# criteo-research/reco-gym

Hardware: AMD Instinct MI355X
Metric: env steps/sec (organic+bandit events emitted/sec), reco-gym-v1 P=10000 K=20 (higher is better)
Workload: dtype f64 (state, click, transition, policy, propensities); organic logits on MFMA as a 2-way fp16 split of fp32 operands (fp32 accumulate), every index certified against f64; 1 GPU; c3: reco-gym-v1 P=10000 K=20 sigma_omega=0.0 policy=ouc; users_per_gpu=10000000, users_total=10000000, log=16 B/row device log + float64 ps side array

## Files before the change

### __graft_entry__.py

```python
import glob
import os
import subprocess
import sys

ROOT = os.path.dirname(os.path.abspath(__file__))
if ROOT not in sys.path:
    sys.path.insert(0, ROOT)

HIPCC = os.environ.get('HIPCC', '/opt/rocm/bin/hipcc')


def _stale(out, deps):
    return (not os.path.exists(out)) or any(os.path.getmtime(d) > os.path.getmtime(out) for d in deps)


UNITS = ['rg_host', 'rg_exact', 'rg_draw_fp32', 'rg_draw_pipelined', 'rg_draw_wide', 'rg_advance', 'rg_walk', 'rg_draw_exacthi', 'rg_draw_lds', 'rg_ope', 'rg_count', 'rg_ope_logreg', 'rg_ope_eg', 'rg_evolve', 'rg_logreg_poly', 'rg_ope_poly', 'rg_ope_recall', 'rg_weight_history', 'rg_bayes_vb', 'rg_nn_ips']
N_PARTS = len(UNITS)
UNIT_FLAGS = {'rg_draw_lds': ['-mllvm', '-amdgpu-mfma-vgpr-form=1']}


def build_deps():
    return sorted(glob.glob(os.path.join(ROOT, 'recogym_amd', 'csrc', '*.hpp')) + glob.glob(os.path.join(ROOT, 'include', '*.h')))


def build(force=False, parts=None, extra_flags=(), out=None):
    csrc = os.path.join(ROOT, 'recogym_amd', 'csrc')
    srcs = [os.path.join(csrc, u + '.hip') for u in UNITS]
    default_out = os.path.join(csrc, 'librecogym_hip.so')
    out = out or default_out
    objdir = os.path.join(csrc, 'build' if out == default_out else 'build_' + os.path.basename(out).replace('.so', ''))
    deps = srcs + build_deps()
    if force or parts or _stale(out, deps):
        os.makedirs(objdir, exist_ok=True)
        todo = list(parts) if parts else list(range(1, N_PARTS + 1))
        for p in range(1, N_PARTS + 1):
            if p not in todo and _stale(os.path.join(objdir, f'part{p}.o'), deps):
                todo.append(p)
        procs = []
        for p in todo:
            cmd = [HIPCC, '--offload-arch=gfx950', '-O3', '-std=c++17', '-fPIC', *UNIT_FLAGS.get(UNITS[p - 1], []), *extra_flags, '-c',
                   '-o', os.path.join(objdir, f'part{p}.o'), srcs[p - 1]]
            procs.append((p, subprocess.Popen(cmd, stderr=open(os.path.join(objdir, f'part{p}.log'), 'w'))))
        for p, pr in procs:
            if pr.wait() != 0:
                sys.stderr.write(open(os.path.join(objdir, f'part{p}.log')).read()[-8000:])
                raise RuntimeError(f'hipcc failed on {UNITS[p - 1]}.hip')
        subprocess.check_call([HIPCC, '--offload-arch=gfx950', '-shared', '-fPIC', '-o', out] +
                              [os.path.join(objdir, f'part{p}.o') for p in range(1, N_PARTS + 1)])
    from oracle import oracle as orc
    orc.build(force=force)
    import recogym_amd
    from recogym_amd import _abi
    _abi.load()
    return out


def smoke():
    import numpy as np
    import torch
    build()
    from oracle import oracle as orc
    from recogym_amd import _abi
    from recogym_amd.envs.configuration import Configuration
    from recogym_amd.envs.reco_env_v1 import env_1_args
    from recogym_amd.sim import Simulator
    assert torch.cuda.is_available(), 'smoke() needs a GPU'
    cfg = Configuration({**env_1_args, 'random_seed': 123, 'num_products': 500, 'K': 20})
    n = 2000
    sim = Simulator(cfg, n, device='cuda:0')
    sim.reset_users(0, n)
    sim.run()
    rows = sim.rows()
    want = orc.OracleEnv(cfg, rng_mode=orc.RNG_PHILOX).generate_logs(n)
    assert len(rows) == len(want), (len(rows), len(want))
    for k in ('u', 't', 'z', 'v', 'a', 'c'):
        assert (rows[k].astype(np.int64) == want[k].astype(np.int64)).all(), k
    c = sim.counters()
    print(f'smoke ok: {len(rows)} rows bit-exact vs oracle; counters {c}')


if __name__ == '__main__':
    _parts = [int(x) for x in sys.argv[sys.argv.index('--parts') + 1].split(',')] if '--parts' in sys.argv else None
    build(force='--force' in sys.argv, parts=_parts)
    if '--smoke' in sys.argv:
        smoke()
```

### recogym_amd/csrc/rg_common.hpp

```cpp

#include <hip/hip_runtime.h>

#include <cmath>
#include <cstdarg>
#include <cstdio>
#include <cstdlib>
#include <cstring>
#include <new>
#include <utility>
#include <vector>

#include "../../include/recogym_hip.h"
#include "../../include/recogym_rng.h"

#pragma once

#ifndef RG_WALK_PRECISE_CHUNK
#define RG_WALK_PRECISE_CHUNK 1
#endif

namespace rgk {

constexpr uint32_t kMaxSteps = 1u << 16;
constexpr int kBlock = 256;
constexpr int kMaxGrid = 4096;
constexpr uint32_t kDefaultHistoryCap = 256;
constexpr uint32_t kPolyListCap = 4096;
constexpr uint32_t kPolySteps = 1024;
constexpr uint32_t kPolyHist = 256;
inline bool lr_family(uint32_t policy) { return policy == RG_POLICY_LOGREG_FROZEN || policy == RG_POLICY_LOGREG_POLY || policy == RG_POLICY_BAYES_VB || policy == RG_POLICY_NN_IPS; }
inline bool lists_unresolved(uint32_t policy) { return policy == RG_POLICY_LOGREG_POLY || policy == RG_POLICY_BAYES_VB || policy == RG_POLICY_NN_IPS; }
constexpr uint64_t kBayesModelBytes = 1ull << 31;
constexpr uint32_t kNnHidden = 1024;
constexpr uint32_t kNnProducts = 4000;
constexpr size_t kNnStageBytes = 48 * 1024;
constexpr size_t kNnStaticLds = 16 * 1024;
constexpr uint64_t kRepackMinUsers = 1ull << 18;

inline thread_local char g_err[512] = "";

inline int fail(int code, const char* fmt, ...) {
    va_list ap;
    va_start(ap, fmt);
    vsnprintf(g_err, sizeof(g_err), fmt, ap);
    va_end(ap);
    return code;
}

#define HIP_TRY(expr)                                                                     \
    do {                                                                                  \
        hipError_t e_ = (expr);                                                           \
        if (e_ != hipSuccess)                                                             \
            return fail(RG_ENODEV, "%s failed: %s", #expr, hipGetErrorString(e_));        \
    } while (0)

inline size_t align_up(size_t x, size_t a) { return (x + a - 1) / a * a; }

struct TpRec { double u; float S, pb, q, dlt; uint32_t ti, pad; };
constexpr uint32_t kTpShards = 16, kTpBins = 128, kTpLists = kTpBins * kTpShards;
__host__ __device__ constexpr uint32_t tp_shards_of(uint32_t n_tiles) {
    uint32_t s = kTpShards;
    while (s < 128u && 2u * s * (n_tiles ? n_tiles : 1u) <= kTpLists) s *= 2u;
    return s;
}
__host__ __device__ constexpr uint32_t tp_rec_stride(uint32_t KH) { return (32u + 8u * KH + 63u) & ~63u; }
inline uint32_t tp_shard_cap(uint64_t n, uint32_t shards) { return static_cast<uint32_t>((((n + 255) / 256 + shards - 1) / shards) * 256); }

struct DevSim {
    uint32_t P, K;
    uint64_t seed, policy_seed;
    double cdf_o0, cdf_o1, cdf_b0, cdf_b1;
    double sigma0, sigma_omega;
    uint32_t change_omega_for_bandits, policy;
    uint32_t ouc_select_randomly, ouc_exploit_explore, ouc_reverse_pop, hist_cap;
    double ouc_epsilon;
    uint64_t first_user;
    uint32_t n_users;
    uint32_t n_cap, n_pad;
    uint64_t organic_only_below;
    const double* gamma; const double* mu_o; const double* beta; const double* mu_b;
    float* gamma32; float* mu32;
    uint32_t has_g32t;
    float* gamma32t;
    double* gammaT;
    uint32_t PT;
    double* gamma_rm;
    uint32_t XKB;
    float* exact_ref;
    double* exact_sums;
    uint32_t exact_rows;
    uint32_t walk_handover;
    uint32_t walk_refill;
    uint32_t walk_bias;
    uint32_t walk_click_batch;
    uint32_t walk_search_batch;
    uint32_t walk_helpers;
    uint32_t walk_click_join;
    uint32_t walk_line64;
    uint32_t exact_base;
    uint32_t exact_last;
    float2* sc_scratch;
    float* chunk_scratch;
    char* tp_rec;
    uint32_t* tp_hist;
    uint32_t* tp_order;
    uint32_t tp_cap, tp_shards;
    uint32_t tp_cpt;
    float* stats;
    uint32_t KH;
    uint32_t KS;
    uint32_t TP;
    uint32_t P_pad;
    uint32_t n_chunks;
    uint32_t sc_chunks;
    uint32_t n_sc;
    uint32_t use_mfma;
    uint32_t N1, N2, N3;
    uint32_t f16;
    uint32_t wide;
    uint32_t RS;
    uint32_t TPB;
    unsigned short* gsplit;
    float* mu32s;
    uint32_t XNH, XNL, XRS;
    unsigned short* xsplit;
    float* xmulo;
    float* xstats;
    uint32_t ablate;
    uint32_t use_cache;
    float2* cache_rec;
    float* cache_chunk;
    float* beta32;
    uint32_t KB4;
    uint8_t* cache_resc;
    float* cache_row; uint32_t cache_row_f;
    float* walk_hot; float* walk_scp;
    uint32_t fin_in_sweep;
    uint32_t sweep_only;
    uint32_t* park_list;
    uint32_t* park_t;
    uint8_t* f64_valid;
    uint32_t grp_lo, grp_n;
    uint32_t list_in;
    unsigned long long* q_ticket;
    unsigned long long* q_park;
    const unsigned long long* q_count;
    unsigned long long* walk_ctl;
    unsigned long long* step1_buf;
    uint32_t* exact_cnt_b;
    double* omega;
    uint32_t OMS;
    uint32_t* list;
    uint32_t* step_cnt;
    uint64_t* log_base;
    uint32_t* exact_list;
    uint32_t* exact_cnt;
    uint32_t run_ahead;
    uint32_t* ev;
    unsigned long long* run_ctl;
    uint32_t* n_events;
    rg_event* phantom;
    uint8_t* has_phantom;
    unsigned long long* hist;
    uint32_t* lpv;
    uint32_t* uid;
    double* omega_alt; unsigned long long* hist_alt; uint32_t* lpv_alt; uint32_t* uid_alt;
// ... 869 lines not shown
    *ps_out = 1.0;
    if (d.policy != RG_POLICY_LOGREG_FROZEN) g = policy_act(d, slot, user, t, ps_out);
    return eg_overlay(d, user, t, g, ps_out);
}

__device__ void history_add(const DevSim& d, uint32_t slot, uint32_t v) {
    if (d.lr_dirty) d.lr_dirty[d.uid[slot]] = 1;
    hent_t* hr = hist_row(d, slot);
    hent_t e[kHistRegs];
    hist_load_line(hr, e);
    const uint32_t nd = h_cnt(e[0]);
    const hent_t key = static_cast<hent_t>(v) << 32;
    if (nd < kHistRegs) {
        uint32_t pos = 1;
        bool hit = false;
#pragma unroll
        for (int i = 1; i < kHistRegs; ++i)
            if (static_cast<uint32_t>(i) <= nd) {
                pos += e[i] < key ? 1u : 0u;
                hit = hit || h_prod(e[i]) == v;
            }
        if (hit) {
#pragma unroll
            for (int i = 1; i < kHistRegs; ++i)
                if (static_cast<uint32_t>(i) == pos) hr[i] = e[i] + 1ull;
            hr[0] = e[0] + (1ull << 32);
            return;
        }
        if (nd + 1 >= d.hist_cap) { atomicAdd(&d.counters[RG_CNT_HIST_OVERFLOW], 1ull); return; }
        hent_t f[kHistRegs + 2];
        f[0] = e[0] + (1ull << 32) + 1ull;
#pragma unroll
        for (int i = 1; i < kHistRegs + 1; ++i)
            f[i] = static_cast<uint32_t>(i) < pos ? e[i < kHistRegs ? i : 0] : (static_cast<uint32_t>(i) == pos ? (key | 1ull) : e[i - 1]);
        f[kHistRegs + 1] = 0ull;
        hr[0] = f[0];
#pragma unroll
        for (int i = 0; i < (kHistRegs + 2) / 2; ++i)
            if (static_cast<uint32_t>(2 * i + 1) >= pos && static_cast<uint32_t>(2 * i) <= nd + 1)
                reinterpret_cast<ulonglong2*>(hr)[i] = make_ulonglong2(i == 0 ? f[0] : f[2 * i], f[2 * i + 1]);
        return;
    }
    if RG_WALK_ABL(22) return;
    uint32_t pos = 1;
    hent_t at = 0ull;
    bool past = false;
    for (uint32_t base = 0; base <= nd && !past; base += kHistRegs) {
        hent_t f[kHistRegs];
        if (base) hist_load_line(hr + base, f);
        else {
#pragma unroll
            for (int i = 0; i < kHistRegs; ++i) f[i] = e[i];
        }
#pragma unroll
        for (int i = 0; i < kHistRegs; ++i) {
            const uint32_t idx = base + i;
            if (idx >= 1 && idx <= nd && !past) {
                if (f[i] < key) pos = idx + 1;
                else { past = true; at = f[i]; }
            }
        }
    }
    if (past && h_prod(at) == v) {
        hr[pos] = at + 1ull;
        hr[0] = e[0] + (1ull << 32);
        return;
    }
    if (nd + 1 >= d.hist_cap) { atomicAdd(&d.counters[RG_CNT_HIST_OVERFLOW], 1ull); return; }
    uint32_t j = nd + 1;
    while (j > pos) {
        if (j >= pos + 4) {
            const hent_t a0 = hr[j - 4], a1 = hr[j - 3], a2 = hr[j - 2], a3 = hr[j - 1];
            hr[j - 3] = a0; hr[j - 2] = a1; hr[j - 1] = a2; hr[j] = a3;
            j -= 4;
        } else { hr[j] = hr[j - 1]; --j; }
    }
    hr[pos] = key | 1ull;
    hr[0] = e[0] + (1ull << 32) + 1ull;
}

__device__ __forceinline__ uint32_t history_tail_add(hent_t* hr, uint32_t nd, uint32_t v, uint32_t first = 16u) {
    const hent_t key = static_cast<hent_t>(v) << 32;
    uint32_t pos = first;
    hent_t at = 0ull;
    bool past = false;
    for (uint32_t base = first; base <= nd && !past; base += kHistRegs) {
        hent_t f[kHistRegs];
        hist_load_line(hr + base, f);
#pragma unroll
        for (int i = 0; i < kHistRegs; ++i) {
            const uint32_t idx = base + i;
            if (idx <= nd && !past) {
                if (f[i] < key) pos = idx + 1;
                else { past = true; at = f[i]; }
            }
        }
    }
    if (past && h_prod(at) == v) { hr[pos] = at + 1ull; return 0u; }
    uint32_t j = nd + 1;
    while (j > pos) {
        if (j >= pos + 4) {
            const hent_t a0 = hr[j - 4], a1 = hr[j - 3], a2 = hr[j - 2], a3 = hr[j - 1];
            hr[j - 3] = a0; hr[j - 2] = a1; hr[j - 1] = a2; hr[j] = a3;
            j -= 4;
        } else { hr[j] = hr[j - 1]; --j; }
    }
    hr[pos] = key | 1ull;
    return 1u;
}

__device__ __forceinline__ double wave_max(double x) {
    for (int o = 32; o > 0; o >>= 1) x = fmax(x, __shfl_xor(x, o));
    return x;
}
__device__ __forceinline__ double wave_sum(double x) {
    for (int o = 32; o > 0; o >>= 1) x += __shfl_xor(x, o);
    return x;
}

__device__ __forceinline__ void write_organic_row(const DevSim& d, uint32_t t, uint32_t pos, uint32_t slot,
                                                  uint32_t user, uint32_t v) {
    const uint64_t row = d.log_base[t] + pos;
    if (d.log && row < d.log_cap) {
        rg_event e;
        e.u = user; e.t = d.run_ahead ? d.ev[d.uid[slot]] : t; e.code = v; e.ps = __builtin_nanf("");
        d.log[row] = e;
        if (d.aux_time) d.aux_time[row] = d.utime[d.uid[slot]];
    }
    if (d.lpv) d.lpv[slot] = v;
}

__device__ __forceinline__ double exp64(double x) {
    x = fmax(x, -750.0);
    const double kf = rint(x * 1.4426950408889634074);
    double r = fma(-kf, 6.93147180369123816490e-01, x);
    r = fma(-kf, 1.90821492927058770002e-10, r);
    double p = 1.6059043836821613e-10;
    p = fma(p, r, 2.08767569878681e-09);
    p = fma(p, r, 2.505210838544172e-08);
    p = fma(p, r, 2.755731922398589e-07);
    p = fma(p, r, 2.7557319223985893e-06);
    p = fma(p, r, 2.48015873015873e-05);
    p = fma(p, r, 1.984126984126984e-04);
    p = fma(p, r, 1.388888888888889e-03);
    p = fma(p, r, 8.333333333333333e-03);
    p = fma(p, r, 4.1666666666666664e-02);
    p = fma(p, r, 1.6666666666666666e-01);
    p = fma(p, r, 0.5);
    p = fma(p, r, 1.0);
    p = fma(p, r, 1.0);
    return ldexp(p, static_cast<int>(kf));
}

static __device__ const double kExp2Tab32[32] = {
    0x1.0000000000000p+0, 0x1.059b0d3158574p+0, 0x1.0b5586cf9890fp+0, 0x1.11301d0125b51p+0,
    0x1.172b83c7d517bp+0, 0x1.1d4873168b9aap+0, 0x1.2387a6e756238p+0, 0x1.29e9df51fdee1p+0,
    0x1.306fe0a31b715p+0, 0x1.371a7373aa9cbp+0, 0x1.3dea64c123422p+0, 0x1.44e086061892dp+0,
    0x1.4bfdad5362a27p+0, 0x1.5342b569d4f82p+0, 0x1.5ab07dd485429p+0, 0x1.6247eb03a5585p+0,
    0x1.6a09e667f3bcdp+0, 0x1.71f75e8ec5f74p+0, 0x1.7a11473eb0187p+0, 0x1.82589994cce13p+0,
    0x1.8ace5422aa0dbp+0, 0x1.93737b0cdc5e5p+0, 0x1.9c49182a3f090p+0, 0x1.a5503b23e255dp+0,
    0x1.ae89f995ad3adp+0, 0x1.b7f76f2fb5e47p+0, 0x1.c199bdd85529cp+0, 0x1.cb720dcef9069p+0,
    0x1.d5818dcfba487p+0, 0x1.dfc97337b9b5fp+0, 0x1.ea4afa2a490dap+0, 0x1.f50765b6e4540p+0};

__device__ __forceinline__ double exp64t(double x, const double* tab) {
    x = fmax(x, -750.0);
    const double nf = rint(x * 0x1.71547652b82fep+5);
    double r = fma(nf, -0x1.62e42fe000000p-6, x);
    r = fma(nf, -0x1.f473de6af278fp-35, r);
    const int n = static_cast<int>(nf);
    double p = 1.3888888888888889e-03;
    p = fma(p, r, 8.3333333333333332e-03);
    p = fma(p, r, 4.1666666666666664e-02);
    p = fma(p, r, 1.6666666666666666e-01);
    p = fma(p, r, 0.5);
    p = fma(p, r, 1.0);
    p = fma(p, r, 1.0);
    return ldexp(tab[n & 31] * p, n >> 5);
}

__device__ __forceinline__ double wave_scan(double x, int lane) {
    for (int o = 1; o < 64; o <<= 1) {
        const double y = __shfl_up(x, o);
        if (lane >= o) x += y;
    }
    return x;
}

__device__ __forceinline__ double logit64(const DevSim& d, const double* om, uint32_t p) {
    const double* g = d.gammaT + p;
    double l = 0.0;
#pragma unroll 4
    for (uint32_t k = 0; k < d.K; ++k) l += g[static_cast<size_t>(k) * d.PT] * om[k];
    return l + d.mu_o[p];
}

__device__ __forceinline__ void logit64x4(const DevSim& d, const double* om, uint32_t p, double out[4]) {
    uint32_t idx[4];
#pragma unroll
    for (int u = 0; u < 4; ++u) { idx[u] = min(p + 64u * u, d.PT - 1); out[u] = 0.0; }
#pragma unroll 2
    for (uint32_t k = 0; k < d.K; ++k) {
        const double w = om[k];
        const double* g = d.gammaT + static_cast<size_t>(k) * d.PT;
#pragma unroll
        for (int u = 0; u < 4; ++u) out[u] += g[idx[u]] * w;
    }
#pragma unroll
    for (int u = 0; u < 4; ++u) out[u] = (p + 64u * u < d.P) ? out[u] + d.mu_o[p + 64u * u] : -INFINITY;
}

constexpr int kUPW = 4;
constexpr int kExactUsers = 4 * kUPW;



using f64x4 = __attribute__((ext_vector_type(4))) double;
__host__ __device__ constexpr int exact_m_groups(uint32_t kb) { return kb <= 8 ? 4 : 2; }
__host__ __device__ constexpr uint32_t exact_m_lds(uint32_t kb) { return (2u * 64u * (4u * kb + 4u) + 32u) * 8u; }


typedef const __attribute__((address_space(4))) double kdouble;


inline void launch_exact_m(exact_m_kernel_t km, const DevSim& d, uint32_t t, int from_list, int mode, uint64_t est, hipStream_t st) {
    const uint32_t upb = (kBlock / 64) * 16 * exact_m_groups(d.XKB);
    const uint64_t groups = (est + upb - 1) / upb;
    const uint32_t n_chunks = d.PT / 64;
    uint32_t S = static_cast<uint32_t>(4096 / (groups ? groups : 1));
    if (S > n_chunks) S = n_chunks;
    if (S < 1) S = 1;
    uint64_t grid = groups * S;
    if (grid > 2048) grid = 2048;
    if (grid < 1) grid = 1;
    const size_t smem = exact_m_lds(d.XKB);
    if (smem > 64 * 1024)
        (void)hipFuncSetAttribute(reinterpret_cast<const void*>(km), hipFuncAttributeMaxDynamicSharedMemorySize, static_cast<int>(smem));
    hipLaunchKernelGGL(km, dim3(static_cast<uint32_t>(grid)), dim3(kBlock), smem, st, d, t, from_list, mode, S);
}



__device__ __forceinline__ uint32_t exact_pick_wave(const DevSim& d, const double* sums, const double* om, double M,
                                                    double u, uint32_t G, int lane, uint32_t om_stride = 1) {
    const uint32_t n_chunks = d.PT / 64;
    const uint32_t n_cc = (n_chunks + G - 1) / G;
    constexpr int RB = 4;
    double x[RB], incl[RB];
    const bool in_regs = n_cc <= 64u * RB;
    double total = 0.0;
    if (in_regs) {
#pragma unroll
        for (int r = 0; r < RB; ++r) {
            const uint32_t c = 64u * r + lane;
            x[r] = c < n_cc ? sums[c] : 0.0;
        }
#pragma unroll
        for (int r = 0; r < RB; ++r) {
            if (64u * r < n_cc) { incl[r] = wave_scan(x[r], lane); total += __shfl(incl[r], 63); }
            else incl[r] = 0.0;
        }
    } else {
        for (uint32_t c0 = 0; c0 < n_cc; c0 += 64) {
            const uint32_t c = c0 + lane;
            total += __shfl(wave_scan(c < n_cc ? sums[c] : 0.0, lane), 63);
        }
    }
    const double target = u * total;
    uint32_t ccstar = n_cc - 1;
    double before = 0.0, run = 0.0;
    bool found = false;
    if (in_regs) {
#pragma unroll
        for (int r = 0; r < RB; ++r) {
            if (64u * r < n_cc && !found) {
                const uint32_t c = 64u * r + lane;
                const unsigned long long hit = __ballot(c < n_cc && run + incl[r] > target);
                if (hit) {
                    const int L = __builtin_ctzll(hit);
                    ccstar = 64u * r + L;
                    before = run + __shfl(incl[r] - x[r], L);
                    found = true;
                } else run += __shfl(incl[r], 63);
            }
        }
    } else {
        for (uint32_t c0 = 0; c0 < n_cc && !found; c0 += 64) {
            const uint32_t c = c0 + lane;
            const double xv = c < n_cc ? sums[c] : 0.0;
            const double inc = wave_scan(xv, lane);
            const unsigned long long hit = __ballot(c < n_cc && run + inc > target);
            if (hit) {
                const int L = __builtin_ctzll(hit);
                ccstar = c0 + L;
                before = run + __shfl(inc - xv, L);
                found = true;
            } else run += __shfl(inc, 63);
        }
    }
    if (!found) before = run - sums[n_cc - 1];
    __builtin_amdgcn_wave_barrier();
    uint32_t v = min(ccstar * G * 64 + G * 64 - 1, d.P - 1);
    double acc = before;
    for (uint32_t i = 0; i < G; ++i) {
        const uint32_t p = (ccstar * G + i) * 64 + lane;
        if (ccstar * G + i >= n_chunks) break;
        const double* g = d.gammaT + p;
        double lg = 0.0;
        for (uint32_t k0 = 0; k0 < d.K; k0 += 8) {
            double gv[8];
#pragma unroll
            for (int j = 0; j < 8; ++j) gv[j] = g[static_cast<size_t>(min(k0 + j, d.K - 1)) * d.PT];
#pragma unroll
            for (int j = 0; j < 8; ++j) if (k0 + j < d.K) lg += gv[j] * om[(k0 + j) * om_stride];
        }
        lg = p < d.P ? lg + d.mu_o[p] : -INFINITY;
        const double inc = wave_scan(exp64(lg - M), lane);
        const unsigned long long hit = __ballot(p < d.P && acc + inc > target);
        if (hit) { v = (ccstar * G + i) * 64 + static_cast<uint32_t>(__builtin_ctzll(hit)); break; }
        acc += __shfl(inc, 63);
    }
    return v;
}


using f32x16 = __attribute__((ext_vector_type(16))) float;

constexpr float kLog2e = 1.44269504088896340736f;
constexpr float kRescaleGap = 57.0f;
constexpr double kDeltaFixed = 3.0e-5;
constexpr double kDeltaPerRescale = 6.0e-6;
constexpr double kDeltaFixedBf16 = 1.0e-5;
// ... 537 lines not shown
```

### recogym_amd/csrc/rg_exact.hip

```cpp

#include "rg_common.hpp"

namespace rgk {

__global__ void __launch_bounds__(kBlock) k_exact_sums(DevSim d, uint32_t t, int from_list, int mode, uint32_t S) {
    extern __shared__ __attribute__((aligned(16))) char smem_raw[];
    const int wave = threadIdx.x >> 6, lane = lane_id();
    const uint32_t n_chunks = d.PT / 64;
    const uint32_t n_cc = (n_chunks + 7) / 8;
    double* g_tile = reinterpret_cast<double*>(smem_raw);
    double* mu_tile = g_tile + static_cast<size_t>(d.K) * 64;
    double* om_all = mu_tile + 64;
    const uint32_t n_o = d.step_cnt[2 * t + RG_STATE_ORGANIC];
    const bool batched = from_list == 1 && !d.use_cache;
    const uint32_t base = batched ? d.exact_base : 0u;
    uint32_t n = from_list ? d.exact_cnt[t] : n_o;
    if (batched) n = min(n, base + d.exact_rows);
    const uint32_t* cur = list_ptr(d, t & 1, RG_STATE_ORGANIC);
    const uint32_t n_groups = n > base ? (n - base + kExactUsers - 1) / kExactUsers : 0u;
    const uint32_t cps = ((n_cc + S - 1) / S) * 8;
    const uint32_t n_work = n_groups * S;

    for (uint32_t wk = blockIdx.x; wk < n_work; wk += gridDim.x) {
        const uint32_t grp = wk / S, slice = wk % S;
        const uint32_t c0 = slice * cps, c1 = min(c0 + cps, n_chunks);
        if (c0 >= c1) continue;
        uint32_t w_idx[kUPW], srow[kUPW];
        bool act[kUPW];
        double M[kUPW], part[kUPW];
#pragma unroll
        for (int u = 0; u < kUPW; ++u) part[u] = 0.0;
        __syncthreads();
        double* om = om_all + static_cast<size_t>(wave * kUPW) * d.K;
#pragma unroll
        for (int u = 0; u < kUPW; ++u) {
            w_idx[u] = base + grp * kExactUsers + wave * kUPW + u;
            act[u] = w_idx[u] < n;
            const uint32_t pos = act[u] ? (from_list ? d.exact_list[w_idx[u]] : w_idx[u]) : 0u;
            const uint32_t slot = act[u] ? cur[pos] : 0u;
            srow[u] = w_idx[u] - base;
            if (from_list && d.use_cache && act[u]) { w_idx[u] = d.uid[slot]; srow[u] = w_idx[u]; }
            M[u] = (mode == 1 && act[u]) ? static_cast<double>(d.exact_ref[w_idx[u]]) * 0.69314718055994530942 : 0.0;
            for (uint32_t k = lane; k < d.K; k += 64)
                om[k * kUPW + u] = act[u] ? d.omega[static_cast<size_t>(slot) * d.OMS + k] : 0.0;
        }
        constexpr int kPF = 8;
        const bool prefetch = d.K * 64 <= kPF * kBlock;
        double pf[kPF];
        double pf_mu = 0.0;
        auto fetch = [&](uint32_t c) {
#pragma unroll
            for (int i = 0; i < kPF; ++i) {
                const uint32_t idx = threadIdx.x + i * kBlock;
                if (idx < d.K * 64) pf[i] = d.gammaT[static_cast<size_t>(idx >> 6) * d.PT + c * 64 + (idx & 63)];
            }
            if (threadIdx.x < 64) { const uint32_t p = c * 64 + threadIdx.x; pf_mu = p < d.P ? d.mu_o[p] : -INFINITY; }
        };
        if (prefetch) fetch(c0);
        for (uint32_t c = c0; c < c1; ++c) {
            __syncthreads();
            if (prefetch) {
#pragma unroll
                for (int i = 0; i < kPF; ++i) {
                    const uint32_t idx = threadIdx.x + i * kBlock;
                    if (idx < d.K * 64) g_tile[idx] = pf[i];
                }
                if (threadIdx.x < 64) mu_tile[threadIdx.x] = pf_mu;
            } else {
                for (uint32_t i = threadIdx.x; i < d.K * 64; i += kBlock) {
                    const uint32_t k = i >> 6, pp = i & 63;
                    g_tile[i] = d.gammaT[static_cast<size_t>(k) * d.PT + c * 64 + pp];
                }
                if (threadIdx.x < 64) {
                    const uint32_t p = c * 64 + threadIdx.x;
                    mu_tile[threadIdx.x] = p < d.P ? d.mu_o[p] : -INFINITY;
                }
            }
            __syncthreads();
            if (prefetch && c + 1 < c1) fetch(c + 1);
            double l[kUPW];
#pragma unroll
            for (int u = 0; u < kUPW; ++u) l[u] = 0.0;
#pragma unroll 4
            for (uint32_t k = 0; k < d.K; ++k) {
                const double g = g_tile[k * 64 + lane];
                const double4 o4 = *reinterpret_cast<const double4*>(om + k * kUPW);
                l[0] += g * o4.x; l[1] += g * o4.y; l[2] += g * o4.z; l[3] += g * o4.w;
            }
            const double mu = mu_tile[lane];
#pragma unroll
            for (int u = 0; u < kUPW; ++u) {
                l[u] += mu;
                part[u] = mode == 0 ? fmax(part[u] == 0.0 && (c & 7) == 0 ? -INFINITY : part[u], l[u])
                                    : part[u] + exp64(l[u] - M[u]);
            }
            if ((c & 7) == 7 || c + 1 == c1) {
#pragma unroll
                for (int u = 0; u < kUPW; ++u) {
                    const double r = mode == 0 ? wave_max(part[u]) : wave_sum(part[u]);
                    if (lane == 0 && act[u]) d.exact_sums[static_cast<size_t>(srow[u]) * n_cc + (c >> 3)] = r;
                    part[u] = 0.0;
                }
            }
        }
    }
}

template <int KB>
__global__ void __launch_bounds__(kBlock) k_exact_sums_m(DevSim d, uint32_t t, int from_list, int mode, uint32_t S) {
    constexpr int G = exact_m_groups(KB);
    constexpr uint32_t UPW = 16 * G, UPB = (kBlock / 64) * UPW;
    constexpr uint32_t RSd = 4 * KB + 4, TILE = 64 * RSd;
    constexpr int NLD = (TILE / 2 + kBlock - 1) / kBlock;
    extern __shared__ __attribute__((aligned(16))) char smem_raw[];
    double* tiles = reinterpret_cast<double*>(smem_raw);
    double* exp_tab = tiles + 2 * TILE;
    if (threadIdx.x < 32) exp_tab[threadIdx.x] = kExp2Tab32[threadIdx.x];
    const int lane = lane_id(), wave = threadIdx.x >> 6;
    const int q = lane >> 4, jl = lane & 15;
    const uint32_t n_cc = d.PT / 64;
    const uint32_t n_o = d.step_cnt[2 * t + RG_STATE_ORGANIC];
    const bool batched = from_list == 1 && !d.use_cache;
    const uint32_t base = batched ? d.exact_base : 0u;
    uint32_t n = from_list == 2 ? t : (from_list ? d.exact_cnt[t] : n_o);
    if (batched) n = min(n, base + d.exact_rows);
    const uint32_t* cur = list_ptr(d, t & 1, RG_STATE_ORGANIC);
    const uint32_t n_groups = n > base ? (n - base + UPB - 1) / UPB : 0u;
    const uint32_t ccps = (n_cc + S - 1) / S;
    const uint32_t n_work = n_groups * S;
    for (uint32_t wk = blockIdx.x; wk < n_work; wk += gridDim.x) {
        const uint32_t grp = wk / S, slice = wk % S;
        const uint32_t cc0 = slice * ccps, cc1 = min(cc0 + ccps, n_cc);
        if (cc0 >= cc1) continue;
        uint32_t row[G];
        bool act[G];
        double b[G][KB], M[G];
#pragma unroll
        for (int g = 0; g < G; ++g) {
            uint32_t w_idx = base + grp * UPB + wave * UPW + g * 16 + jl;
            act[g] = w_idx < n;
            uint32_t slot;
            if (from_list == 2) {
                slot = act[g] ? d.park_list[w_idx] : 0xFFFFFFFFu;
                act[g] = slot != 0xFFFFFFFFu;
                if (!act[g]) slot = 0u;
                w_idx = slot;
            } else {
                const uint32_t pos = act[g] ? (from_list ? d.exact_list[w_idx] : w_idx) : 0u;
                slot = act[g] ? cur[pos] : 0u;
                if (from_list && d.use_cache && act[g]) w_idx = d.uid[slot];
            }
            row[g] = w_idx - (batched ? base : 0u);
#pragma unroll
            for (int s2 = 0; s2 < KB; ++s2) {
                const uint32_t k = 4 * s2 + q;
                b[g][s2] = (act[g] && k < d.K) ? d.omega[static_cast<size_t>(slot) * d.OMS + k] : 0.0;
            }
            M[g] = (mode == 1 && act[g]) ? static_cast<double>(d.exact_ref[w_idx]) * 0.69314718055994530942 : 0.0;
        }
        double2 pf[NLD];
        auto fetch = [&](uint32_t cc) {
            const double2* src = reinterpret_cast<const double2*>(d.gamma_rm + static_cast<size_t>(cc) * TILE);
#pragma unroll
            for (int i = 0; i < NLD; ++i) {
                const uint32_t idx = threadIdx.x + i * kBlock;
                if (idx < TILE / 2) pf[i] = src[idx];
            }
        };
        auto stash = [&](uint32_t buf) {
            double2* dst = reinterpret_cast<double2*>(tiles + buf * TILE);
#pragma unroll
            for (int i = 0; i < NLD; ++i) {
                const uint32_t idx = threadIdx.x + i * kBlock;
                if (idx < TILE / 2) dst[idx] = pf[i];
            }
        };
        __syncthreads();
        fetch(cc0);
        stash(0);
        for (uint32_t cc = cc0; cc < cc1; ++cc) {
            __syncthreads();
            const bool more = cc + 1 < cc1;
            if (more) fetch(cc + 1);
            const double* A = tiles + ((cc - cc0) & 1u) * TILE;
            double sum[G];
#pragma unroll
            for (int g = 0; g < G; ++g) sum[g] = mode == 0 ? -INFINITY : 0.0;
#pragma unroll 1
            for (int tt = 0; tt < 4; ++tt) {
                f64x4 acc[G];
#pragma unroll
                for (int g = 0; g < G; ++g) acc[g] = f64x4{0.0, 0.0, 0.0, 0.0};
                const double* arow = A + static_cast<size_t>(tt * 16 + jl) * RSd + q;
#pragma unroll
                for (int s2 = 0; s2 < KB; ++s2) {
                    const double a = arow[4 * s2];
#pragma unroll
                    for (int g = 0; g < G; ++g) acc[g] = __builtin_amdgcn_mfma_f64_16x16x4f64(a, b[g][s2], acc[g], 0, 0, 0);
                }
                double mu[4];
#pragma unroll
                for (int r = 0; r < 4; ++r) mu[r] = A[static_cast<size_t>(tt * 16 + q + 4 * r) * RSd + 4 * KB];
#pragma unroll
                for (int g = 0; g < G; ++g)
#pragma unroll
                    for (int r = 0; r < 4; ++r) {
                        const double l = acc[g][r] + mu[r];
                        sum[g] = mode == 0 ? fmax(sum[g], l) : sum[g] + exp64t(l - M[g], exp_tab);
                    }
            }
#pragma unroll
            for (int g = 0; g < G; ++g) {
                double x = sum[g];
                const double y = __shfl_xor(x, 16);
                x = mode == 0 ? fmax(x, y) : x + y;
                const double z = __shfl_xor(x, 32);
                x = mode == 0 ? fmax(x, z) : x + z;
                if (q == (g & 3) && act[g]) d.exact_sums[static_cast<size_t>(row[g]) * n_cc + cc] = x;
            }
            if (more) stash(((cc - cc0) & 1u) ^ 1u);
        }
    }
}

template <int KB>
__global__ void __launch_bounds__(kBlock) k_exact_sums_h(DevSim d, uint32_t n, uint32_t mfma_of_8) {
    constexpr int G = exact_m_groups(KB);
    constexpr uint32_t UPW = 16 * G, UPB = (kBlock / 64) * UPW;
    constexpr uint32_t RSd = 4 * KB + 4, TILE = 64 * RSd;
    constexpr int NLD = (TILE / 2 + kBlock - 1) / kBlock;
    extern __shared__ __attribute__((aligned(16))) char smem_raw[];
    double* tiles = reinterpret_cast<double*>(smem_raw);
    double* exp_tab = tiles + 2 * TILE;
    __shared__ uint32_t s_grp;
    if (threadIdx.x < 32) exp_tab[threadIdx.x] = kExp2Tab32[threadIdx.x];
    const int lane = lane_id(), wave = threadIdx.x >> 6;
    const int q = lane >> 4, jl = lane & 15;
    const uint32_t n_cc = d.PT / 64;
    if (d.q_count) n = static_cast<uint32_t>(*d.q_count);
    const uint32_t* plist = d.park_list + d.list_in;
    const uint32_t n_groups = (n + UPB - 1) / UPB;
    uint32_t S = 1;
    if (n_groups && n_groups < 16u * gridDim.x) S = min(8u, (16u * gridDim.x + n_groups - 1) / n_groups);
    S = min(S, n_cc);
    const uint32_t n_items = n_groups * S;
    for (;;) {
        __syncthreads();
        if (threadIdx.x == 0) s_grp = static_cast<uint32_t>(atomicAdd(d.q_ticket, 1ull));
        __syncthreads();
        if (s_grp >= n_items) break;
        const uint32_t grp = s_grp / S, slice = s_grp % S;
        const uint32_t cc_lo = slice * n_cc / S, cc_hi = (slice + 1u) * n_cc / S;
        if ((grp & 7u) < mfma_of_8) {
            uint32_t row[G];
            bool act[G];
            double b[G][KB], M[G];
#pragma unroll
            for (int g = 0; g < G; ++g) {
                const uint32_t w_idx = grp * UPB + wave * UPW + g * 16 + jl;
                uint32_t slot = w_idx < n ? plist[w_idx] : 0xFFFFFFFFu;
                act[g] = slot != 0xFFFFFFFFu;
                if (!act[g]) slot = 0u;
                row[g] = slot;
#pragma unroll
                for (int s2 = 0; s2 < KB; ++s2) {
                    const uint32_t k = 4 * s2 + q;
                    b[g][s2] = (act[g] && k < d.K) ? d.omega[static_cast<size_t>(slot) * d.OMS + k] : 0.0;
                }
                M[g] = act[g] ? static_cast<double>(d.exact_ref[slot]) * 0.69314718055994530942 : 0.0;
            }
            double2 pf[NLD];
            auto fetch = [&](uint32_t cc) {
                const double2* src = reinterpret_cast<const double2*>(d.gamma_rm + static_cast<size_t>(cc) * TILE);
#pragma unroll
                for (int i = 0; i < NLD; ++i) {
                    const uint32_t idx = threadIdx.x + i * kBlock;
                    if (idx < TILE / 2) pf[i] = src[idx];
                }
            };
            auto stash = [&](uint32_t buf) {
                double2* dst = reinterpret_cast<double2*>(tiles + buf * TILE);
#pragma unroll
                for (int i = 0; i < NLD; ++i) {
                    const uint32_t idx = threadIdx.x + i * kBlock;
                    if (idx < TILE / 2) dst[idx] = pf[i];
                }
            };
            fetch(cc_lo);
            stash(cc_lo & 1u);
            for (uint32_t cc = cc_lo; cc < cc_hi; ++cc) {
                __syncthreads();
                const bool more = cc + 1 < cc_hi;
                if (more) fetch(cc + 1);
                const double* A = tiles + (cc & 1u) * TILE;
                double sum[G];
#pragma unroll
                for (int g = 0; g < G; ++g) sum[g] = 0.0;
#pragma unroll 1
                for (int tt = 0; tt < 4; ++tt) {
                    f64x4 acc[G];
#pragma unroll
                    for (int g = 0; g < G; ++g) acc[g] = f64x4{0.0, 0.0, 0.0, 0.0};
                    const double* arow = A + static_cast<size_t>(tt * 16 + jl) * RSd + q;
#pragma unroll
                    for (int s2 = 0; s2 < KB; ++s2) {
                        const double a = arow[4 * s2];
#pragma unroll
                        for (int g = 0; g < G; ++g) acc[g] = __builtin_amdgcn_mfma_f64_16x16x4f64(a, b[g][s2], acc[g], 0, 0, 0);
                    }
                    double mu[4];
#pragma unroll
                    for (int r = 0; r < 4; ++r) mu[r] = A[static_cast<size_t>(tt * 16 + q + 4 * r) * RSd + 4 * KB];
#pragma unroll
                    for (int g = 0; g < G; ++g)
#pragma unroll
                        for (int r = 0; r < 4; ++r) sum[g] += exp64t(acc[g][r] + mu[r] - M[g], exp_tab);
                }
#pragma unroll
                for (int g = 0; g < G; ++g) {
                    double x = sum[g];
                    x += __shfl_xor(x, 16);
                    x += __shfl_xor(x, 32);
                    if (q == (g & 3) && act[g]) d.exact_sums[static_cast<size_t>(row[g]) * n_cc + cc] = x;
                }
                if (more) stash((cc & 1u) ^ 1u);
            }
        } else {
            constexpr int UPL = UPB / (kBlock / 64) / 64;
            uint32_t w_row[UPL];
            bool act[UPL];
            double om[UPL][4 * KB], M[UPL];
#pragma unroll
            for (int j = 0; j < UPL; ++j) {
                const uint32_t w_idx = grp * UPB + wave * 64 * UPL + j * 64 + lane;
                uint32_t slot = w_idx < n ? plist[w_idx] : 0xFFFFFFFFu;
                act[j] = slot != 0xFFFFFFFFu;
                if (!act[j]) slot = 0u;
                w_row[j] = slot;
#pragma unroll
                for (int k = 0; k < 4 * KB; ++k)
                    om[j][k] = (act[j] && static_cast<uint32_t>(k) < d.K) ? d.omega[static_cast<size_t>(slot) * d.OMS + k] : 0.0;
                M[j] = act[j] ? static_cast<double>(d.exact_ref[slot]) * 0.69314718055994530942 : 0.0;
            }
            for (uint32_t cc = cc_lo; cc < cc_hi; ++cc) {
                double acc[UPL];
#pragma unroll
                for (int j = 0; j < UPL; ++j) acc[j] = 0.0;
                const uint32_t p1 = cc * 64 + 64;
#pragma unroll 2
                for (uint32_t p = cc * 64; p < p1; ++p) {
                    kdouble* row = (kdouble*)(d.gamma_rm) + static_cast<size_t>(p) * RSd;
                    double l[UPL];
#pragma unroll
                    for (int j = 0; j < UPL; ++j) l[j] = 0.0;
#pragma unroll
                    for (int k = 0; k < 4 * KB; ++k) {
                        const double g = row[k];
#pragma unroll
                        for (int j = 0; j < UPL; ++j) l[j] += g * om[j][k];
                    }
#pragma unroll
                    for (int j = 0; j < UPL; ++j) acc[j] += exp64t(l[j] + row[4 * KB] - M[j], exp_tab);
                }
#pragma unroll
                for (int j = 0; j < UPL; ++j)
                    if (act[j]) d.exact_sums[static_cast<size_t>(w_row[j]) * n_cc + cc] = acc[j];
            }
        }
    }
}

exact_h_kernel_t exact_h_kernel_for(uint32_t kb) {
    switch (kb) {
        case 1: return k_exact_sums_h<1>;   case 2: return k_exact_sums_h<2>;   case 3: return k_exact_sums_h<3>;
        case 4: return k_exact_sums_h<4>;   case 5: return k_exact_sums_h<5>;   case 6: return k_exact_sums_h<6>;
        case 8: return k_exact_sums_h<8>;
        default: return nullptr;
    }
}

exact_m_kernel_t exact_m_kernel_for(uint32_t kb) {
    switch (kb) {
        case 1: return k_exact_sums_m<1>;   case 2: return k_exact_sums_m<2>;   case 3: return k_exact_sums_m<3>;
        case 4: return k_exact_sums_m<4>;   case 5: return k_exact_sums_m<5>;   case 6: return k_exact_sums_m<6>;
        case 8: return k_exact_sums_m<8>;   case 12: return k_exact_sums_m<12>; case 16: return k_exact_sums_m<16>;
        default: return nullptr;
    }
}

__global__ void __launch_bounds__(kBlock) k_exact_ref(DevSim d, uint32_t t, uint32_t G) {
    const int lane = lane_id();
    const uint32_t n_cc = (d.PT / 64 + G - 1) / G;
    const uint32_t n = d.step_cnt[2 * t + RG_STATE_ORGANIC];
    const uint32_t waves_total = gridDim.x * (kBlock / 64);
    for (uint32_t w = blockIdx.x * (kBlock / 64) + (threadIdx.x >> 6); w < n; w += waves_total) {
        double m = -INFINITY;
        for (uint32_t c = lane; c < n_cc; c += 64) m = fmax(m, d.exact_sums[static_cast<size_t>(w) * n_cc + c]);
        m = wave_max(m);
        if (lane == 0) d.exact_ref[w] = static_cast<float>(m * 1.4426950408889634074);
    }
}

__global__ void __launch_bounds__(kBlock) k_exact_pick(DevSim d, uint32_t t, int from_list, uint32_t G) {
    extern __shared__ __attribute__((aligned(16))) char smem_raw[];
    const int wave = threadIdx.x >> 6, lane = lane_id();
    double* om = reinterpret_cast<double*>(smem_raw) + static_cast<size_t>(wave) * d.K;
    const uint32_t n_cc = (d.PT / 64 + G - 1) / G;
    const uint32_t n_o = d.step_cnt[2 * t + RG_STATE_ORGANIC];
    const bool cached = from_list && d.use_cache;
    const bool batched = from_list == 1 && !d.use_cache;
    const uint32_t base = batched ? d.exact_base : 0u;
    const uint32_t n_all = from_list ? d.exact_cnt[t] : n_o;
    const uint32_t n_a = batched ? min(n_all, base + d.exact_rows) : n_all;
    const uint32_t n = n_a + (cached ? d.exact_cnt_b[t] : 0u);
    const uint32_t* cur = list_ptr(d, t & 1, RG_STATE_ORGANIC);
    const uint32_t waves_total = gridDim.x * (kBlock / 64);
    if (batched && d.exact_last && n_all > n_a && blockIdx.x == 0 && threadIdx.x == 0)
        atomicAdd(&d.counters[RG_CNT_EXACT_OVERFLOW], static_cast<unsigned long long>(n_all - n_a));
    for (uint32_t w = base + blockIdx.x * (kBlock / 64) + wave; w < n; w += waves_total) {
        const uint32_t pos = from_list ? d.exact_list[w < n_a ? w : d.n_cap - 1u - (w - n_a)] : w;
        const uint32_t slot = cur[pos];
        const uint32_t uidx = d.uid[slot];
        const uint32_t user = static_cast<uint32_t>(d.first_user + uidx);
        const uint32_t row = cached ? uidx : w;
        const double M = static_cast<double>(d.exact_ref[row]) * 0.69314718055994530942;
        const double* sums = d.exact_sums + static_cast<size_t>(row - base) * n_cc;
        for (uint32_t k = lane; k < d.K; k += 64) om[k] = d.omega[static_cast<size_t>(slot) * d.OMS + k];
        __builtin_amdgcn_fence(__ATOMIC_ACQ_REL, "workgroup");
        __builtin_amdgcn_wave_barrier();
        const uint32_t v = exact_pick_wave(d, sums, om, M, organic_uniform(d, uidx, user, t), G, lane);
        if (lane == 0) {
            write_organic_row(d, t, pos, slot, user, v);
            if (d.hist_cap) history_add(d, slot, v);
            if (cached && w < n_a) d.f64_valid[uidx] = 1;
        }
        __builtin_amdgcn_wave_barrier();
    }
    if (from_list == 1 && blockIdx.x == 0 && threadIdx.x == 0) {
        atomicAdd(&d.counters[RG_CNT_EXACT_DRAWS], static_cast<unsigned long long>(n > base ? n - base : 0u));
        atomicAdd(&d.counters[RG_CNT_EXACT_SWEEPS], static_cast<unsigned long long>(n_a > base ? n_a - base : 0u));
    }
}
exact_m_kernel_t exact_tile_kernel() { return k_exact_sums; }
exact_h_kernel_t exact_ref_kernel() { return k_exact_ref; }
exact_pick_kernel_t exact_pick_kernel() { return k_exact_pick; }

}
```

Measured before the change: 10.07 billion events/s.

## Rework exact-sum exp path: bit-trick exp, bias-in-MFMA accumulator, pipelined row loads

Replaces the table exp with a version that forms the 2^n scale by integer-adding the exponent into a pre-biased table entry. This drops the ldexp and rint/convert work, and the final multiply-add is fused into the accumulation. The MFMA accumulators are seeded with mu-M so the bias is folded into the matrix op. The scalar fallback path double-buffers gamma rows with scheduling barriers so loads overlap the dot+exp work. It also enables the mfma-vgpr-form flag for the exact unit. Risks: the clamp changes from -750 to -708, which affects denormal/underflow results, and seeding the accumulator with the bias changes rounding order.

```diff
diff --git a/__graft_entry__.py b/__graft_entry__.py
--- a/__graft_entry__.py
+++ b/__graft_entry__.py
@@ -16,7 +16,7 @@
 
 UNITS = ['rg_host', 'rg_exact', 'rg_draw_fp32', 'rg_draw_pipelined', 'rg_draw_wide', 'rg_advance', 'rg_walk', 'rg_draw_exacthi', 'rg_draw_lds', 'rg_ope', 'rg_count', 'rg_ope_logreg', 'rg_ope_eg', 'rg_evolve', 'rg_logreg_poly', 'rg_ope_poly', 'rg_ope_recall', 'rg_weight_history', 'rg_bayes_vb', 'rg_nn_ips']
 N_PARTS = len(UNITS)
-UNIT_FLAGS = {'rg_draw_lds': ['-mllvm', '-amdgpu-mfma-vgpr-form=1']}
+UNIT_FLAGS = {'rg_draw_lds': ['-mllvm', '-amdgpu-mfma-vgpr-form=1'], 'rg_exact': ['-mllvm', '-amdgpu-mfma-vgpr-form=1']}
 
 
 def build_deps():
diff --git a/recogym_amd/csrc/rg_common.hpp b/recogym_amd/csrc/rg_common.hpp
--- a/recogym_amd/csrc/rg_common.hpp
+++ b/recogym_amd/csrc/rg_common.hpp
@@ -12,6 +12,7 @@
 
 #include "../../include/recogym_hip.h"
 #include "../../include/recogym_rng.h"
+#include "rg_exp64.hpp"
 
 #pragma once
 
@@ -1187,31 +1188,6 @@
     return ldexp(p, static_cast<int>(kf));
 }
 
-static __device__ const double kExp2Tab32[32] = {
-    0x1.0000000000000p+0, 0x1.059b0d3158574p+0, 0x1.0b5586cf9890fp+0, 0x1.11301d0125b51p+0,
-    0x1.172b83c7d517bp+0, 0x1.1d4873168b9aap+0, 0x1.2387a6e756238p+0, 0x1.29e9df51fdee1p+0,
-    0x1.306fe0a31b715p+0, 0x1.371a7373aa9cbp+0, 0x1.3dea64c123422p+0, 0x1.44e086061892dp+0,
-    0x1.4bfdad5362a27p+0, 0x1.5342b569d4f82p+0, 0x1.5ab07dd485429p+0, 0x1.6247eb03a5585p+0,
-    0x1.6a09e667f3bcdp+0, 0x1.71f75e8ec5f74p+0, 0x1.7a11473eb0187p+0, 0x1.82589994cce13p+0,
-    0x1.8ace5422aa0dbp+0, 0x1.93737b0cdc5e5p+0, 0x1.9c49182a3f090p+0, 0x1.a5503b23e255dp+0,
-    0x1.ae89f995ad3adp+0, 0x1.b7f76f2fb5e47p+0, 0x1.c199bdd85529cp+0, 0x1.cb720dcef9069p+0,
-    0x1.d5818dcfba487p+0, 0x1.dfc97337b9b5fp+0, 0x1.ea4afa2a490dap+0, 0x1.f50765b6e4540p+0};
-
-__device__ __forceinline__ double exp64t(double x, const double* tab) {
-    x = fmax(x, -750.0);
-    const double nf = rint(x * 0x1.71547652b82fep+5);
-    double r = fma(nf, -0x1.62e42fe000000p-6, x);
-    r = fma(nf, -0x1.f473de6af278fp-35, r);
-    const int n = static_cast<int>(nf);
-    double p = 1.3888888888888889e-03;
-    p = fma(p, r, 8.3333333333333332e-03);
-    p = fma(p, r, 4.1666666666666664e-02);
-    p = fma(p, r, 1.6666666666666666e-01);
-    p = fma(p, r, 0.5);
-    p = fma(p, r, 1.0);
-    p = fma(p, r, 1.0);
-    return ldexp(tab[n & 31] * p, n >> 5);
-}
 
 __device__ __forceinline__ double wave_scan(double x, int lane) {
     for (int o = 1; o < 64; o <<= 1) {
diff --git a/recogym_amd/csrc/rg_exact.hip b/recogym_amd/csrc/rg_exact.hip
--- a/recogym_amd/csrc/rg_exact.hip
+++ b/recogym_amd/csrc/rg_exact.hip
@@ -114,8 +114,8 @@
     constexpr int NLD = (TILE / 2 + kBlock - 1) / kBlock;
     extern __shared__ __attribute__((aligned(16))) char smem_raw[];
     double* tiles = reinterpret_cast<double*>(smem_raw);
-    double* exp_tab = tiles + 2 * TILE;
-    if (threadIdx.x < 32) exp_tab[threadIdx.x] = kExp2Tab32[threadIdx.x];
+    uint32_t* exp_tab = reinterpret_cast<uint32_t*>(tiles + 2 * TILE);
+    if (threadIdx.x < 32) exp64t_entry(kExp2Tab32[threadIdx.x], threadIdx.x, exp_tab);
     const int lane = lane_id(), wave = threadIdx.x >> 6;
     const int q = lane >> 4, jl = lane & 15;
     const uint32_t n_cc = d.PT / 64;
@@ -188,9 +188,14 @@
             for (int g = 0; g < G; ++g) sum[g] = mode == 0 ? -INFINITY : 0.0;
 #pragma unroll 1
             for (int tt = 0; tt < 4; ++tt) {
+                double mu[4];
+#pragma unroll
+                for (int r = 0; r < 4; ++r) mu[r] = A[static_cast<size_t>(tt * 16 + q + 4 * r) * RSd + 4 * KB];
                 f64x4 acc[G];
 #pragma unroll
-                for (int g = 0; g < G; ++g) acc[g] = f64x4{0.0, 0.0, 0.0, 0.0};
+                for (int g = 0; g < G; ++g)
+#pragma unroll
+                    for (int r = 0; r < 4; ++r) acc[g][r] = mu[r] - M[g];
                 const double* arow = A + static_cast<size_t>(tt * 16 + jl) * RSd + q;
 #pragma unroll
                 for (int s2 = 0; s2 < KB; ++s2) {
@@ -198,16 +203,11 @@
 #pragma unroll
                     for (int g = 0; g < G; ++g) acc[g] = __builtin_amdgcn_mfma_f64_16x16x4f64(a, b[g][s2], acc[g], 0, 0, 0);
                 }
-                double mu[4];
-#pragma unroll
-                for (int r = 0; r < 4; ++r) mu[r] = A[static_cast<size_t>(tt * 16 + q + 4 * r) * RSd + 4 * KB];
 #pragma unroll
                 for (int g = 0; g < G; ++g)
 #pragma unroll
-                    for (int r = 0; r < 4; ++r) {
-                        const double l = acc[g][r] + mu[r];
-                        sum[g] = mode == 0 ? fmax(sum[g], l) : sum[g] + exp64t(l - M[g], exp_tab);
-                    }
+                    for (int r = 0; r < 4; ++r)
+                        sum[g] = mode == 0 ? fmax(sum[g], acc[g][r]) : exp64t_add(sum[g], acc[g][r], exp_tab);
             }
 #pragma unroll
             for (int g = 0; g < G; ++g) {
@@ -231,9 +231,9 @@
     constexpr int NLD = (TILE / 2 + kBlock - 1) / kBlock;
     extern __shared__ __attribute__((aligned(16))) char smem_raw[];
     double* tiles = reinterpret_cast<double*>(smem_raw);
-    double* exp_tab = tiles + 2 * TILE;
+    uint32_t* exp_tab = reinterpret_cast<uint32_t*>(tiles + 2 * TILE);
     __shared__ uint32_t s_grp;
-    if (threadIdx.x < 32) exp_tab[threadIdx.x] = kExp2Tab32[threadIdx.x];
+    if (threadIdx.x < 32) exp64t_entry(kExp2Tab32[threadIdx.x], threadIdx.x, exp_tab);
     const int lane = lane_id(), wave = threadIdx.x >> 6;
     const int q = lane >> 4, jl = lane & 15;
     const uint32_t n_cc = d.PT / 64;
@@ -298,9 +298,14 @@
                 for (int g = 0; g < G; ++g) sum[g] = 0.0;
 #pragma unroll 1
                 for (int tt = 0; tt < 4; ++tt) {
+                    double mu[4];
+#pragma unroll
+                    for (int r = 0; r < 4; ++r) mu[r] = A[static_cast<size_t>(tt * 16 + q + 4 * r) * RSd + 4 * KB];
                     f64x4 acc[G];
 #pragma unroll
-                    for (int g = 0; g < G; ++g) acc[g] = f64x4{0.0, 0.0, 0.0, 0.0};
+                    for (int g = 0; g < G; ++g)
+#pragma unroll
+                        for (int r = 0; r < 4; ++r) acc[g][r] = mu[r] - M[g];
                     const double* arow = A + static_cast<size_t>(tt * 16 + jl) * RSd + q;
 #pragma unroll
                     for (int s2 = 0; s2 < KB; ++s2) {
@@ -308,13 +313,10 @@
 #pragma unroll
                         for (int g = 0; g < G; ++g) acc[g] = __builtin_amdgcn_mfma_f64_16x16x4f64(a, b[g][s2], acc[g], 0, 0, 0);
                     }
-                    double mu[4];
-#pragma unroll
-                    for (int r = 0; r < 4; ++r) mu[r] = A[static_cast<size_t>(tt * 16 + q + 4 * r) * RSd + 4 * KB];
 #pragma unroll
                     for (int g = 0; g < G; ++g)
 #pragma unroll
-                        for (int r = 0; r < 4; ++r) sum[g] += exp64t(acc[g][r] + mu[r] - M[g], exp_tab);
+                        for (int r = 0; r < 4; ++r) sum[g] = exp64t_add(sum[g], acc[g][r], exp_tab);
                 }
 #pragma unroll
                 for (int g = 0; g < G; ++g) {
@@ -327,6 +329,8 @@
             }
         } else {
             constexpr int UPL = UPB / (kBlock / 64) / 64;
+            constexpr int RW = 4 * KB + 1;
+            constexpr bool kTwoRows = 4 * RW <= 84;
             uint32_t w_row[UPL];
             bool act[UPL];
             double om[UPL][4 * KB], M[UPL];
@@ -342,29 +346,70 @@
                     om[j][k] = (act[j] && static_cast<uint32_t>(k) < d.K) ? d.omega[static_cast<size_t>(slot) * d.OMS + k] : 0.0;
                 M[j] = act[j] ? static_cast<double>(d.exact_ref[slot]) * 0.69314718055994530942 : 0.0;
             }
-            for (uint32_t cc = cc_lo; cc < cc_hi; ++cc) {
-                double acc[UPL];
-#pragma unroll
-                for (int j = 0; j < UPL; ++j) acc[j] = 0.0;
-                const uint32_t p1 = cc * 64 + 64;
-#pragma unroll 2
-                for (uint32_t p = cc * 64; p < p1; ++p) {
-                    kdouble* row = (kdouble*)(d.gamma_rm) + static_cast<size_t>(p) * RSd;
-                    double l[UPL];
-#pragma unroll
-                    for (int j = 0; j < UPL; ++j) l[j] = 0.0;
-#pragma unroll
-                    for (int k = 0; k < 4 * KB; ++k) {
-                        const double g = row[k];
-#pragma unroll
-                        for (int j = 0; j < UPL; ++j) l[j] += g * om[j][k];
+            auto dot_exp = [&](const double (&r)[RW], double (&scale)[UPL], double (&poly)[UPL]) {
+#pragma unroll
+                for (int j = 0; j < UPL; ++j) {
+                    double l = r[4 * KB] - M[j];
+#pragma unroll
+                    for (int k = 0; k < 4 * KB; ++k) l = fma(r[k], om[j][k], l);
+                    exp64t_parts(l, exp_tab, scale[j], poly[j]);
+                }
+            };
+            auto load_row = [&](double (&r)[RW], uint32_t p) {
+                kdouble* row = (kdouble*)(d.gamma_rm) + static_cast<size_t>(p) * RSd;
+#pragma unroll
+                for (int k = 0; k < RW; ++k) r[k] = row[k];
+            };
+            if constexpr (kTwoRows) {
+                const uint32_t p_last = cc_hi * 64 - 1;
+                double ra[RW], rb[RW];
+                load_row(ra, cc_lo * 64);
+                load_row(rb, cc_lo * 64 + 1);
+#pragma unroll
+                for (int k = 0; k < RW; k += 4) asm volatile("" ::"s"(ra[k]), "s"(rb[k]));
+                auto step = [&](double (&r)[RW], uint32_t p_next, double (&acc)[UPL]) {
+                    double scale[UPL], poly[UPL];
+                    dot_exp(r, scale, poly);
+                    __builtin_amdgcn_sched_barrier(0);
+                    load_row(r, min(p_next, p_last));
+                    __builtin_amdgcn_sched_barrier(0);
+#pragma unroll
+                    for (int j = 0; j < UPL; ++j) acc[j] = fma(scale[j], poly[j], acc[j]);
+                };
+                for (uint32_t cc = cc_lo; cc < cc_hi; ++cc) {
+                    double acc[UPL];
+#pragma unroll
+                    for (int j = 0; j < UPL; ++j) acc[j] = 0.0;
+                    const uint32_t p1 = cc * 64 + 64;
+#pragma unroll 1
+                    for (uint32_t p = cc * 64; p < p1; p += 2) {
+                        step(ra, p + 2, acc);
+                        step(rb, p + 3, acc);
                     }
 #pragma unroll
-                    for (int j = 0; j < UPL; ++j) acc[j] += exp64t(l[j] + row[4 * KB] - M[j], exp_tab);
-                }
-#pragma unroll
-                for (int j = 0; j < UPL; ++j)
-                    if (act[j]) d.exact_sums[static_cast<size_t>(w_row[j]) * n_cc + cc] = acc[j];
+                    for (int j = 0; j < UPL; ++j)
+                        if (act[j]) d.exact_sums[static_cast<size_t>(w_row[j]) * n_cc + cc] = acc[j];
+                }
+            } else {
+                for (uint32_t cc = cc_lo; cc < cc_hi; ++cc) {
+                    double acc[UPL];
+#pragma unroll
+                    for (int j = 0; j < UPL; ++j) acc[j] = 0.0;
+                    const uint32_t p1 = cc * 64 + 64;
+#pragma unroll 1
+                    for (uint32_t p = cc * 64; p < p1; p += 2)
+#pragma unroll
+                        for (uint32_t h = 0; h < 2; ++h) {
+                            double r[RW], scale[UPL], poly[UPL];
+                            load_row(r, p + h);
+                            dot_exp(r, scale, poly);
+#pragma unroll
+                            for (int j = 0; j < UPL; ++j) acc[j] = fma(scale[j], poly[j], acc[j]);
+                        }
+#pragma unroll
+                    for (int j = 0; j < UPL; ++j)
+                        if (act[j]) d.exact_sums[static_cast<size_t>(w_row[j]) * n_cc + cc] = acc[j];
+                }
             }
         }
     }
diff --git a/recogym_amd/csrc/rg_exp64.hpp b/recogym_amd/csrc/rg_exp64.hpp
--- /dev/null
+++ b/recogym_amd/csrc/rg_exp64.hpp
@@ -0,0 +1,54 @@
+#pragma once
+
+#include <cstdint>
+
+#if defined(__HIPCC__)
+#define RG_EXP64_HD __host__ __device__ __forceinline__
+#define RG_EXP64_TABLE static __device__ const
+#else
+#define RG_EXP64_HD inline
+#define RG_EXP64_TABLE static const
+#endif
+
+RG_EXP64_TABLE double kExp2Tab32[32] = {
+    0x1.0000000000000p+0, 0x1.059b0d3158574p+0, 0x1.0b5586cf9890fp+0, 0x1.11301d0125b51p+0,
+    0x1.172b83c7d517bp+0, 0x1.1d4873168b9aap+0, 0x1.2387a6e756238p+0, 0x1.29e9df51fdee1p+0,
+    0x1.306fe0a31b715p+0, 0x1.371a7373aa9cbp+0, 0x1.3dea64c123422p+0, 0x1.44e086061892dp+0,
+    0x1.4bfdad5362a27p+0, 0x1.5342b569d4f82p+0, 0x1.5ab07dd485429p+0, 0x1.6247eb03a5585p+0,
+    0x1.6a09e667f3bcdp+0, 0x1.71f75e8ec5f74p+0, 0x1.7a11473eb0187p+0, 0x1.82589994cce13p+0,
+    0x1.8ace5422aa0dbp+0, 0x1.93737b0cdc5e5p+0, 0x1.9c49182a3f090p+0, 0x1.a5503b23e255dp+0,
+    0x1.ae89f995ad3adp+0, 0x1.b7f76f2fb5e47p+0, 0x1.c199bdd85529cp+0, 0x1.cb720dcef9069p+0,
+    0x1.d5818dcfba487p+0, 0x1.dfc97337b9b5fp+0, 0x1.ea4afa2a490dap+0, 0x1.f50765b6e4540p+0};
+
+RG_EXP64_HD void exp64t_entry(double tj, uint32_t j, uint32_t* tab) {
+    const uint64_t bits = __builtin_bit_cast(uint64_t, tj) - (static_cast<uint64_t>(j) << 47);
+    tab[2 * j] = static_cast<uint32_t>(bits);
+    tab[2 * j + 1] = static_cast<uint32_t>(bits >> 32);
+}
+
+RG_EXP64_HD void exp64t_parts(double x, const uint32_t* tab, double& scale, double& poly) {
+    x = __builtin_fmax(x, -708.0);
+    const double t = __builtin_fma(x, 0x1.71547652b82fep+5, 0x1.8p52);
+    const uint32_t n = static_cast<uint32_t>(__builtin_bit_cast(uint64_t, t));
+    const double nf = t - 0x1.8p52;
+    double r = __builtin_fma(nf, -0x1.62e42fe000000p-6, x);
+    r = __builtin_fma(nf, -0x1.f473de6af278fp-35, r);
+    double p = 1.3888888888888889e-03;
+    p = __builtin_fma(p, r, 8.3333333333333332e-03);
+    p = __builtin_fma(p, r, 4.1666666666666664e-02);
+    p = __builtin_fma(p, r, 1.6666666666666666e-01);
+    p = __builtin_fma(p, r, 0.5);
+    p = __builtin_fma(p, r, 1.0);
+    poly = __builtin_fma(p, r, 1.0);
+    const uint32_t* w = tab + ((n & 31u) << 1);
+    const uint32_t lo = w[0], hi = w[1] + (n << 15);
+    scale = __builtin_bit_cast(double, (static_cast<uint64_t>(hi) << 32) | lo);
+}
+
+RG_EXP64_HD double exp64t_add(double sum, double x, const uint32_t* tab) {
+    double scale, poly;
+    exp64t_parts(x, tab, scale, poly);
+    return __builtin_fma(scale, poly, sum);
+}
+
+RG_EXP64_HD double exp64t(double x, const uint32_t* tab) { return exp64t_add(0.0, x, tab); }
```

After: 10.25 billion events/s, median of 6. 1.7% higher.
